# sparisi/pvr_habitat

Measured on AMD Instinct MI355X. Metric: frames/sec embedded (ResNet50, 256x256), higher is better.
Workload: dtype f16; 1 GPU; configs[1]: ResNet50 (MoCo-v2 layout) frozen, 256x256 uint8 frames resident in HBM, batch 256/GPU, random-init synthetic weights, f16 storage / MFMA inputs with fp32 accumulation (the product default, inside the 1e-3 parity bound; configs[1] names bf16); global_batch=256, frame=256, chunk=256, batches_in_flight=2, parallelism=frame shards, no collective (dp1)

## Files before the change

include/pvr_hip.h:

```cpp
#ifndef PVR_HIP_H
#define PVR_HIP_H

#include <stddef.h>
#include <stdint.h>

#ifdef __cplusplus
extern "C" {
#endif

typedef int pvr_status;
#define PVR_OK 0
#define PVR_ERR_INVALID 1
#define PVR_ERR_MISSING_WEIGHT 2
#define PVR_ERR_HIP 3
#define PVR_ERR_STATE 4

#define PVR_BF16 0
#define PVR_F16 1
#define PVR_F32 2

#define PVR_ARCH_RESNET50 0
#define PVR_ARCH_RESNET50_L4 1
#define PVR_ARCH_RESNET50_L3 2
#define PVR_ARCH_CLIP_VIT_B32 3
// ... 53 lines not shown
int32_t pvr_encoder_launch_kernel(const pvr_encoder *enc, int32_t n, int32_t index, char *buf, int32_t cap);
void pvr_encoder_destroy(pvr_encoder *enc);

pvr_status pvr_op_preprocess(const uint8_t *frames_dev, int32_t n, int32_t h, int32_t w, int32_t resize,
                             int32_t crop, void *out_dev, int32_t dtype, void *hip_stream);
pvr_status pvr_op_stem(const void *img_dev, const void *wgt_dev, const float *bias_dev, void *out_dev,
                       int32_t n, int32_t dtype, void *hip_stream);
pvr_status pvr_op_maxpool(const void *in_dev, void *out_dev, int32_t n, int32_t h, int32_t w, int32_t c,
                          int32_t dtype, void *hip_stream);
pvr_status pvr_op_conv2d(const void *in_dev, const void *wgt_dev, const float *bias_dev,
                         const void *residual_dev, void *out_dev, int32_t n, int32_t h, int32_t w,
                         int32_t cin, int32_t cout, int32_t kh, int32_t kw, int32_t stride, int32_t pad,
                         int32_t relu, int32_t out_f32, int32_t dtype, void *hip_stream);
pvr_status pvr_op_bneck_frame(const void *t1_dev, const void *w2_dev, const float *b2_dev, const void *w3_dev, const float *b3_dev,
                              const void *residual_dev, void *y_dev, void *t2_out_dev, const void *w1n_dev, const float *b1n_dev, void *t1n_dev,
                              const void *w1f_dev, const float *b1f_dev, int32_t n, int32_t phases, int32_t dtype, void *hip_stream);
pvr_status pvr_op_pack_frag_weights(const void *w_dev, void *out_dev, int32_t rows, int32_t k, void *hip_stream);
pvr_status pvr_debug_bneck_frame_stamps(const void *t1_dev, const void *w2_dev, const float *b2_dev, const void *w3_dev, const float *b3_dev,
                                        const void *residual_dev, void *y_dev, const void *w1n_dev, const float *b1n_dev, void *t1n_dev,
                                        const void *w1f_dev, const float *b1f_dev, int32_t n, int32_t dtype, uint64_t *stamps_dev, void *hip_stream);
int64_t pvr_debug_bneck_frame_launches(void);
pvr_status pvr_debug_set_frame64(int32_t mode);
int64_t pvr_debug_bneck_frame64_launches(void);
pvr_status pvr_debug_bneck_frame64_stamps(const void *w1f_dev, const float *b1f_dev, const void *w2_dev, const float *b2_dev, const void *w3_dev, const float *b3_dev,
                                          const void *x_dev, void *y_dev, int32_t n, int32_t dtype, uint64_t *stamps_dev, void *hip_stream);
pvr_status pvr_op_conv_wfrag(const void *in_dev, const void *wgt_packed_dev, const float *bias_dev, const void *residual_dev, void *out_dev, int32_t n,
                             int32_t h, int32_t w, int32_t cin, int32_t cout, int32_t kh, int32_t kw, int32_t stride, int32_t pad, int32_t relu,
                             int32_t out_f32, int32_t dtype, void *hip_stream);
pvr_status pvr_op_conv2d_dual(const void *in_dev, const void *in2_dev, const void *wgt_dev, const float *bias_dev, void *out_dev, int32_t n, int32_t h,
                              int32_t w, int32_t cin, int32_t cout, int32_t kh, int32_t kw, int32_t stride, int32_t pad, int32_t h2, int32_t w2,
                              int32_t cin2, int32_t stride2, int32_t relu, int32_t dtype, void *hip_stream);
pvr_status pvr_op_conv_wfrag_pool(const void *in_dev, const void *wgt_packed_dev, const float *bias_dev, const void *residual_dev, float *pool_out_dev,
                                  int64_t pool_stride, int32_t n, int32_t cin, int32_t cout, int32_t dtype, void *hip_stream);
int64_t pvr_debug_conv_wfrag_launches(void);
pvr_status pvr_op_split16_pack_weights(const float *w_dev, void *out_dev, int32_t rows, int32_t k, void *hip_stream);
pvr_status pvr_op_conv2d_split16(const float *in_dev, const void *wgt_split_dev, const float *bias_dev, const float *residual_dev, float *out_dev, int32_t n,
                                 int32_t h, int32_t w, int32_t cin, int32_t cout, int32_t k, int32_t stride, int32_t pad, int32_t relu, void *hip_stream);
pvr_status pvr_op_conv2d_f32(const float *in_dev, const float *wgt_dev, const float *bias_dev, const float *residual_dev, float *out_dev, int32_t n,
                             int32_t h, int32_t w, int32_t cin, int32_t cout, int32_t k, int32_t stride, int32_t pad, int32_t relu, void *hip_stream);
int64_t pvr_debug_conv_split16_launches(void);
int64_t pvr_debug_chain_wave128_launches(void);
pvr_status pvr_debug_set_conv_algo(int32_t algo);
pvr_status pvr_file_sizes(const char *const *paths, int32_t n, int64_t *sizes, int32_t threads);
pvr_status pvr_read_files(const char *const *paths, int32_t n, uint8_t *dst, const int64_t *offsets, int32_t threads);
pvr_status pvr_stage_copy(void *dst, const void *src, int64_t rows, int64_t row_bytes, int64_t src_row_stride, int64_t run_bytes,
                          int64_t run_stride, int32_t threads);
int64_t pvr_png_scratch_bytes(int32_t n, int32_t h, int32_t w);
pvr_status pvr_png_decode(const uint8_t *files_dev, const int64_t *offsets_dev, int32_t n, int32_t h, int32_t w, uint8_t *out_dev,
                          uint8_t *scratch_dev, int64_t scratch_bytes, int32_t *status_dev, void *hip_stream);

int64_t pvr_debug_conv_expand_launches(void);
int64_t pvr_debug_pp_persistent_launches(void);
pvr_status pvr_op_avgpool(const void *in_dev, float *out_dev, int64_t out_stride, int32_t n, int32_t hw,
                          int32_t c, int32_t in_f32, int32_t dtype, void *hip_stream);
pvr_status pvr_op_nonfinite_flag(const float *x_dev, int64_t rows, int64_t cols, int64_t stride, int32_t *flag_dev, void *hip_stream);

pvr_status pvr_op_attention(const void *qkv_dev, void *out_dev, int32_t T, int32_t W, int32_t heads, int32_t nb, int32_t dtype, void *hip_stream);
pvr_status pvr_op_layernorm(const float *x_dev, const float *patch_emb_dev, const float *cls_dev, const float *pos_dev, const float *gamma_dev,
                            const float *beta_dev, float *out_f32_dev, void *out_h_dev, int32_t rows, int32_t T, int32_t W, float eps, int32_t normalize,
                            int32_t dtype, void *hip_stream);
pvr_status pvr_op_cls_head(const float *x_dev, const float *gamma_dev, const float *beta_dev, const float *proj_or_null_dev, float *out_dev,
                           int64_t out_stride, int32_t nb, int32_t T, int32_t W, int32_t out_dim, float eps, void *hip_stream);

pvr_status pvr_debug_convert(const float *src, uint16_t *dst, int64_t n, int32_t dtype);


// ... 5 lines not shown
```

pvr_habitat_amd/_lib.py:

```python
import ctypes as C
import os

_HERE = os.path.dirname(os.path.abspath(__file__))
LIB_PATH = os.environ.get('PVR_LIB') or os.path.join(_HERE, 'lib', 'libpvr_hip.so')

PVR_BF16, PVR_F16, PVR_F32 = 0, 1, 2
ARCH_RESNET50, ARCH_RESNET50_L4, ARCH_RESNET50_L3 = 0, 1, 2


class EncoderDesc(C.Structure):
    _fields_ = [('arch', C.c_int32), ('dtype', C.c_int32), ('max_batch', C.c_int32), ('chunk', C.c_int32),
                ('resize', C.c_int32), ('crop', C.c_int32), ('mean', C.c_float * 3), ('std_', C.c_float * 3)]


_lib = None

_SIGS = {
    'pvr_version': (C.c_char_p, []),
    'pvr_has_experiments': (C.c_int32, []),
    'pvr_debug_stem_u8_geometry_ok': (C.c_int32, [C.c_void_p, C.c_int32, C.c_int32, C.c_int32, C.c_int32]),
    'pvr_encoder_set_host_backend': (C.c_int, [C.c_void_p, C.c_int32]),
    'pvr_stage_copy': (C.c_int, [C.c_void_p, C.c_void_p, C.c_int64, C.c_int64, C.c_int64, C.c_int64, C.c_int64, C.c_int32]),
    'pvr_last_error': (C.c_size_t, [C.c_char_p, C.c_size_t]),
    'pvr_encoder_create': (C.c_int, [C.POINTER(EncoderDesc), C.POINTER(C.c_void_p)]),
# ... 4 lines not shown
    'pvr_encoder_forward_lane': (C.c_int, [C.c_void_p, C.c_int32, C.c_void_p, C.c_int32, C.c_int32, C.c_int32, C.c_void_p, C.c_int64, C.c_void_p]),
    'pvr_debug_set_conv_algo': (C.c_int, [C.c_int32]),
    'pvr_file_sizes': (C.c_int, [C.c_void_p, C.c_int32, C.c_void_p, C.c_int32]),
    'pvr_read_files': (C.c_int, [C.c_void_p, C.c_int32, C.c_void_p, C.c_void_p, C.c_int32]),
    'pvr_png_scratch_bytes': (C.c_int64, [C.c_int32, C.c_int32, C.c_int32]),
    'pvr_png_decode': (C.c_int, [C.c_void_p, C.c_void_p, C.c_int32, C.c_int32, C.c_int32, C.c_void_p, C.c_void_p, C.c_int64, C.c_void_p, C.c_void_p]),
    'pvr_debug_conv_expand_launches': (C.c_int64, []),
    'pvr_debug_pp_persistent_launches': (C.c_int64, []),
    'pvr_encoder_set_crop_position': (C.c_int, [C.c_void_p, C.c_int32]),
    'pvr_encoder_set_low_latency': (C.c_int, [C.c_void_p, C.c_int32]),
    'pvr_encoder_tap': (C.c_int, [C.c_void_p, C.c_char_p, C.c_void_p, C.c_int64, C.POINTER(C.c_int64), C.c_void_p]),
    'pvr_encoder_debug_stop_after': (C.c_int, [C.c_void_p, C.c_char_p]),
    'pvr_encoder_debug_set_fusion': (C.c_int, [C.c_void_p, C.c_int32]),
    'pvr_encoder_launch_name': (C.c_int32, [C.c_void_p, C.c_int32, C.c_char_p, C.c_int32]),
    'pvr_encoder_destroy': (None, [C.c_void_p]),
    'pvr_encoder_profile': (C.c_int, [C.c_void_p, C.c_void_p, C.c_int32, C.c_int32, C.c_int32, C.c_void_p, C.c_int64, C.c_void_p,
                                      C.c_void_p, C.c_void_p, C.c_int32, C.POINTER(C.c_int32)]),
    'pvr_encoder_profile_span': (C.c_int, [C.c_void_p, C.c_void_p, C.c_int32, C.c_int32, C.c_int32, C.c_void_p, C.c_int64, C.c_void_p, C.c_int32, C.c_int32,
                                           C.POINTER(C.c_float)]),
    'pvr_op_preprocess': (C.c_int, [C.c_void_p, C.c_int32, C.c_int32, C.c_int32, C.c_int32, C.c_int32, C.c_void_p, C.c_int32, C.c_void_p]),
    'pvr_op_stem': (C.c_int, [C.c_void_p, C.c_void_p, C.c_void_p, C.c_void_p, C.c_int32, C.c_int32, C.c_void_p]),
    'pvr_op_maxpool': (C.c_int, [C.c_void_p, C.c_void_p, C.c_int32, C.c_int32, C.c_int32, C.c_int32, C.c_int32, C.c_void_p]),
    'pvr_op_conv2d': (C.c_int, [C.c_void_p, C.c_void_p, C.c_void_p, C.c_void_p, C.c_void_p] + [C.c_int32] * 12 + [C.c_void_p]),
    'pvr_op_avgpool': (C.c_int, [C.c_void_p, C.c_void_p, C.c_int64, C.c_int32, C.c_int32, C.c_int32, C.c_int32, C.c_int32, C.c_void_p]),
    'pvr_debug_convert': (C.c_int, [C.c_void_p, C.c_void_p, C.c_int64, C.c_int32]),
    'pvr_op_bneck_frame': (C.c_int, [C.c_void_p] * 13 + [C.c_int32] * 3 + [C.c_void_p]),
    'pvr_debug_bneck_frame_launches': (C.c_int64, []),
    'pvr_debug_set_frame64': (C.c_int, [C.c_int32]),
    'pvr_debug_bneck_frame64_launches': (C.c_int64, []),
    'pvr_debug_bneck_frame64_stamps': (C.c_int, [C.c_void_p] * 8 + [C.c_int32] * 2 + [C.c_void_p] * 2),
    'pvr_op_conv_wfrag': (C.c_int, [C.c_void_p] * 5 + [C.c_int32] * 12 + [C.c_void_p]),
    'pvr_debug_conv_wfrag_launches': (C.c_int64, []),
    'pvr_op_conv_wfrag_pool': (C.c_int, [C.c_void_p] * 5 + [C.c_int64] + [C.c_int32] * 4 + [C.c_void_p]),
    'pvr_op_conv2d_dual': (C.c_int, [C.c_void_p] * 5 + [C.c_int32] * 15 + [C.c_void_p]),
    'pvr_op_pack_frag_weights': (C.c_int, [C.c_void_p, C.c_void_p, C.c_int32, C.c_int32, C.c_void_p]),
    'pvr_debug_bneck_frame_stamps': (C.c_int, [C.c_void_p] * 12 + [C.c_int32] * 2 + [C.c_void_p] * 2),
    'pvr_encoder_check_range': (C.c_int, [C.c_void_p, C.c_void_p, C.c_int32, C.c_int32, C.c_int32, C.c_void_p, C.c_int64, C.c_void_p, C.POINTER(C.c_int32)]),
    'pvr_encoder_debug_set_switch': (C.c_int, [C.c_void_p, C.c_char_p, C.c_int32]),
    'pvr_encoder_launch_kernel': (C.c_int32, [C.c_void_p, C.c_int32, C.c_int32, C.c_char_p, C.c_int32]),
    'pvr_op_split16_pack_weights': (C.c_int, [C.c_void_p, C.c_void_p, C.c_int32, C.c_int32, C.c_void_p]),
    'pvr_op_conv2d_split16': (C.c_int, [C.c_void_p] * 5 + [C.c_int32] * 9 + [C.c_void_p]),
    'pvr_op_conv2d_f32': (C.c_int, [C.c_void_p] * 5 + [C.c_int32] * 9 + [C.c_void_p]),
    'pvr_debug_conv_split16_launches': (C.c_int64, []),
    'pvr_debug_chain_wave128_launches': (C.c_int64, []),
    'pvr_op_attention': (C.c_int, [C.c_void_p, C.c_void_p, C.c_int32, C.c_int32, C.c_int32, C.c_int32, C.c_int32, C.c_void_p]),
    'pvr_op_layernorm': (C.c_int, [C.c_void_p] * 8 + [C.c_int32] * 3 + [C.c_float, C.c_int32, C.c_int32, C.c_void_p]),
    'pvr_op_cls_head': (C.c_int, [C.c_void_p] * 5 + [C.c_int64] + [C.c_int32] * 4 + [C.c_float, C.c_void_p]),
    'pvr_op_nonfinite_flag': (C.c_int, [C.c_void_p, C.c_int64, C.c_int64, C.c_int64, C.c_void_p, C.c_void_p]),
}


def lib():
    global _lib
    if _lib is None:
        if not os.path.isfile(LIB_PATH):
            raise RuntimeError('libpvr_hip.so not found at %s: build it with `make -C pvr_habitat_amd/csrc` '
                               '(there is no CPU fallback for the HIP path)' % LIB_PATH)
        l = C.CDLL(LIB_PATH)
        for name, (res, args) in _SIGS.items():
            if not hasattr(l, name):
                continue
            f = getattr(l, name)
            f.restype, f.argtypes = res, args
        _lib = l
    return _lib

# ... 22 lines not shown
```

pvr_habitat_amd/csrc/api.hip:

```cpp
#include <stdarg.h>
#include "encoder_internal.h"
#include "sample_rng.h"
#include <dlfcn.h>

namespace pvr {

static thread_local std::string g_err;

void set_error(const char *fmt, ...) {
    char buf[1024];
    va_list ap;
    va_start(ap, fmt);
    vsnprintf(buf, sizeof buf, fmt, ap);
    va_end(ap);
    g_err = buf;
}
const std::string &last_error() { return g_err; }

namespace {
typedef int (*roctx_push_fn)(const char *);
typedef int (*roctx_pop_fn)();
struct Roctx {
    roctx_push_fn push = nullptr;
    roctx_pop_fn pop = nullptr;
// ... 65 lines not shown
                              w1n, b1n, t1n, w1f, b1f);
}
pvr_status pvr_debug_set_frame64(int32_t mode) {
    PVR_REQUIRE(mode >= -1 && mode <= 1, "pvr_debug_set_frame64: -1 (environment: PVR_FRAME64, default off), 0 or 1");
    if (mode < 0) { PlanSwitches env; read_switches(env); mode = env.frame64; }
    op_switches().frame64 = mode;
    return PVR_OK;
}
int64_t pvr_debug_bneck_frame64_launches(void) { return (int64_t)bneck_frame64_launches(); }
pvr_status pvr_debug_bneck_frame64_stamps(const void *w1f, const float *b1f, const void *w2, const float *b2, const void *w3, const float *b3, const void *x, void *y,
                                          int32_t n, int32_t dtype, uint64_t *stamps_dev, void *stream) {
    PVR_REQUIRE(stamps_dev && n > 8, "pvr_debug_bneck_frame64_stamps: needs a stamp buffer and more than 8 frames");
    return launch_bneck_frame64(w1f, b1f, w2, b2, w3, b3, x, y, n, dtype, (hipStream_t)stream, (unsigned long long *)stamps_dev);
}
pvr_status pvr_op_conv_wfrag(const void *in, const void *wgt_packed, const float *bias, const void *residual, void *out, int32_t n, int32_t h, int32_t w,
                             int32_t cin, int32_t cout, int32_t kh, int32_t kw, int32_t stride, int32_t pad, int32_t relu, int32_t out_f32, int32_t dtype,
                             void *stream) {
    PVR_REQUIRE(n > 0 && h > 0 && w > 0, "pvr_op_conv_wfrag: empty input");
    return launch_conv_wfrag(op_switches(), in, wgt_packed, bias, residual, out, n, h, w, cin, cout, kh, kw, stride, pad, relu, out_f32, dtype, (hipStream_t)stream);
}
pvr_status pvr_op_conv2d_dual(const void *in, const void *in2, const void *wgt, const float *bias, void *out, int32_t n, int32_t h, int32_t w, int32_t cin,
                              int32_t cout, int32_t kh, int32_t kw, int32_t stride, int32_t pad, int32_t h2, int32_t w2, int32_t cin2, int32_t stride2,
                              int32_t relu, int32_t dtype, void *stream) {
    PVR_REQUIRE(in && in2 && wgt && bias && out && n > 0, "pvr_op_conv2d_dual: null argument");
    PVR_REQUIRE(dtype == PVR_BF16 || dtype == PVR_F16, "pvr_op_conv2d_dual: 16-bit storage types only");
    return launch_conv_pp256(op_switches(), in, wgt, bias, nullptr, out, n, h, w, cin, cout, kh, kw, stride, pad, relu, 0, 0, dtype, 224, (hipStream_t)stream, in2, h2, w2,
                             cin2, stride2);
}
pvr_status pvr_op_conv_wfrag_pool(const void *in, const void *wgt_packed, const float *bias, const void *residual, float *pool_out, int64_t pool_stride,
                                  int32_t n, int32_t cin, int32_t cout, int32_t dtype, void *stream) {
    PVR_REQUIRE(n > 0 && pool_out, "pvr_op_conv_wfrag_pool: empty input");
    return launch_conv_wfrag(op_switches(), in, wgt_packed, bias, residual, nullptr, n, 7, 7, cin, cout, 1, 1, 1, 0, 1, 1, dtype, (hipStream_t)stream, pool_out, pool_stride);
}
int64_t pvr_debug_conv_wfrag_launches(void) { return (int64_t)conv_wfrag_launches(); }
pvr_status pvr_op_split16_pack_weights(const float *w, void *out, int32_t rows, int32_t k, void *stream) {
    return launch_split16_pack(w, out, rows, k, (hipStream_t)stream);
}
pvr_status pvr_op_conv2d_split16(const float *in, const void *wgt_split, const float *bias, const float *residual, float *out, int32_t n, int32_t h,
                                 int32_t w, int32_t cin, int32_t cout, int32_t k, int32_t stride, int32_t pad, int32_t relu, void *stream) {
    PVR_REQUIRE(n > 0 && h > 0 && w > 0, "pvr_op_conv2d_split16: empty input");
    return launch_conv_split16(in, wgt_split, bias, residual, out, n, h, w, cin, cout, k, stride, pad, relu, (hipStream_t)stream);
}
pvr_status pvr_op_conv2d_f32(const float *in, const float *wgt, const float *bias, const float *residual, float *out, int32_t n, int32_t h, int32_t w,
                             int32_t cin, int32_t cout, int32_t k, int32_t stride, int32_t pad, int32_t relu, void *stream) {
    PVR_REQUIRE(in && wgt && bias && out && n > 0, "pvr_op_conv2d_f32: null argument");
    return launch_conv_f32(in, wgt, bias, residual, out, n, h, w, cin, cout, k, stride, pad, relu, (hipStream_t)stream);
}
int64_t pvr_debug_conv_split16_launches(void) { return (int64_t)conv_split16_launches(); }
int64_t pvr_debug_chain_wave128_launches(void) { return (int64_t)chain_wave128_launches(); }
int64_t pvr_debug_pp_persistent_launches(void) { return (int64_t)pp_persistent_launches(); }

size_t pvr_last_error(char *buf, size_t cap) {
    const std::string &e = last_error();
    if (buf && cap) {
        size_t n = e.size() < cap - 1 ? e.size() : cap - 1;
        memcpy(buf, e.data(), n);
        buf[n] = 0;
    }
    return e.size();
}

pvr_status pvr_op_preprocess(const uint8_t *frames, int32_t n, int32_t h, int32_t w, int32_t resize, int32_t crop,
                             void *out, int32_t dtype, void *stream) {
    PVR_REQUIRE(frames && out, "pvr_op_preprocess: null pointer");
    hipStream_t st = (hipStream_t)stream;
    PVR_HIP_TRY(hipMemsetAsync(out, 0, (size_t)n * (crop + 6) * (crop + 8) * 4 * 2, st));
// ... 95 lines not shown
```

pvr_habitat_amd/csrc/conv_wfrag.hip:

```cpp
#include "encoder_internal.h"

namespace pvr {

struct WFP {
    const u16 *in, *w, *res;
    const float *bias;
    void *out;
    int M, H, W, Cin, Cout, Ho, Wo, KH, KW, stride, pad, act;
    int MT, NCT;
    int nch, cpt;
    int KC;
    int ct_major;
    unsigned in_bytes, w_bytes, out_bytes, res_bytes;
    float *pool_out;
    long long pool_stride;
    int frames;
};

#define WF_LDS_PTR(off_) ((__attribute__((address_space(3))) void *)(smem + (off_)))

template <bool F16, int RES, bool OUT32, int KO = 0, bool POOL = false>
__global__ __launch_bounds__(512, 1) void conv_wfrag_kernel(WFP p) {
    typedef typename HT<F16>::V8 V8;
    constexpr int BMV = POOL ? 98 : 112;
    constexpr int BM = 112, NT = 7, XB = 16384;
    constexpr int OOB = 0x7ffffff0;
    extern __shared__ __attribute__((aligned(16))) char smem[];

    const int tid = threadIdx.x, lane = tid & 63;
    const int wave = __builtin_amdgcn_readfirstlane(tid >> 6);
    const int fr = lane & 15, fq = lane >> 4, sw = (fr >> 1) & 7;
    const int t = xcd_remap(blockIdx.x, gridDim.x);
    int mt, ct;
    if (p.ct_major) { ct = t / p.MT; mt = t - ct * p.MT; }
    else { mt = t / p.NCT; ct = t - mt * p.NCT; }
    const int m0 = mt * BMV, co0 = ct * 256;

    const auto rs_in = __builtin_amdgcn_make_buffer_rsrc(const_cast<u16 *>(p.in), 0, p.in_bytes, 0x00020000);
    const auto rs_w = __builtin_amdgcn_make_buffer_rsrc(const_cast<u16 *>(p.w), 0, p.w_bytes, 0x00020000);

    int a_off[2], a_m[2];
#pragma unroll
    for (int i = 0; i < 2; ++i) {
        const int g = wave + 8 * i, r = g * 8 + (lane >> 3);
        const int lch = (lane & 7) ^ ((r >> 1) & 7);
        const int m = m0 + r;
        const bool ok = g < BM / 8 && r < BMV && m < p.M;
        const int mm = ok ? m : 0;
        const int wo = mm % p.Wo, tq = mm / p.Wo, ho = tq % p.Ho, n = tq / p.Ho;
// ... 163 lines not shown
    if constexpr (POOL) {
#pragma unroll
        for (int f = 0; f < 2; ++f) {
            float tot[8];
#pragma unroll
            for (int e = 0; e < 8; ++e) {
                float t = ps[f][e];
                if (f == 1) t = __builtin_bit_cast(float, __builtin_amdgcn_update_dpp(0, __builtin_bit_cast(int, t), 0x12f, 0xf, 0xf, false));
                t += __builtin_bit_cast(float, __builtin_amdgcn_update_dpp(0, __builtin_bit_cast(int, t), 0x111, 0xf, 0xf, true));
                t += __builtin_bit_cast(float, __builtin_amdgcn_update_dpp(0, __builtin_bit_cast(int, t), 0x112, 0xf, 0xf, true));
                t += __builtin_bit_cast(float, __builtin_amdgcn_update_dpp(0, __builtin_bit_cast(int, t), 0x114, 0xf, 0xf, true));
                t += __builtin_bit_cast(float, __builtin_amdgcn_update_dpp(0, __builtin_bit_cast(int, t), 0x118, 0xf, 0xf, true));
                tot[e] = t / 49.f;
            }
            const int frame = 2 * mt + f;
            if (fr == 15 && frame < p.frames) {
                float *o = p.pool_out + (long long)frame * p.pool_stride + c;
                *reinterpret_cast<f32x4 *>(o) = f32x4{tot[0], tot[1], tot[2], tot[3]};
                *reinterpret_cast<f32x4 *>(o + 4) = f32x4{tot[4], tot[5], tot[6], tot[7]};
            }
        }
    }
#undef WF_ITER
#undef WF_STEP
#undef WF_XREAD
#undef WF_LOAD_W1
#undef WF_LOAD_W_
#undef WF_LOAD_W
#undef WF_STAGE
#undef WF_STAGE1
#undef WF_STAGE_NEXT
}

static long long g_conv_wfrag_launches = 0;
long long conv_wfrag_launches() { return g_conv_wfrag_launches; }

bool conv_wfrag_supported(int64_t M, int64_t in_bytes, int cin, int cout, int kh, int kw, int pad, int act, int out_f32) {
    const int64_t K = (int64_t)kh * kw * cin;
    return cin % 64 == 0 && cout % 256 == 0 && kh <= 3 && kh == kw && (pad == kh / 2 || pad == 0) && (act == 0 || act == 1) && !(out_f32 & 2) && M >= 1 &&
           M * cout * ((out_f32 & 1) ? 4 : 2) < 0x7ffffff0ll && in_bytes < 0x7ffffff0ll && (int64_t)cout * K * 2 < 0x7ffffff0ll;
}

bool conv_wfrag_preferred(const PlanSwitches &sw, int64_t M, int cin, int cout, int kh, int kw) {
    const int on = sw.conv_wfrag;
    const int64_t K = (int64_t)kh * kw * cin, nct = cout / 256, t256 = ((M + 255) / 256) * nct, t112 = ((M + 111) / 112) * nct;
    if (on == 2) return K >= 512;
    return on && K >= 1024 && t256 < 160 && t112 >= 192;
}

pvr_status launch_conv_wfrag(const PlanSwitches &sw, const void *in, const void *wp, const float *bias, const void *res, void *out, int n, int h, int w, int cin, int cout,
                             int kh, int kw, int stride, int pad, int act, int out_f32, int dtype, hipStream_t stream, float *pool_out, int64_t pool_stride) {
    PVR_REQUIRE(in && wp && bias && (out || pool_out), "conv_wfrag: null argument");
    PVR_REQUIRE(dtype == PVR_BF16 || dtype == PVR_F16, "conv_wfrag: 16-bit storage types only");
    const int ho = (h + 2 * pad - kh) / stride + 1, wo = (w + 2 * pad - kw) / stride + 1;
    const int64_t M = (int64_t)n * ho * wo;
    PVR_REQUIRE(conv_wfrag_supported(M, (int64_t)n * h * w * cin * 2, cin, cout, kh, kw, pad, act, out_f32), "conv_wfrag: unsupported shape");
    WFP p;
    p.in = (const u16 *)in; p.w = (const u16 *)wp; p.res = (const u16 *)res; p.bias = bias; p.out = out;
    p.M = (int)M; p.H = h; p.W = w; p.Cin = cin; p.Cout = cout; p.Ho = ho; p.Wo = wo; p.KH = kh; p.KW = kw; p.stride = stride; p.pad = pad; p.act = act;
    p.MT = pool_out ? (n + 1) / 2 : (int)((M + 111) / 112); p.NCT = cout / 256;
    p.pool_out = pool_out; p.pool_stride = pool_stride; p.frames = n;
    PVR_REQUIRE(!pool_out || (ho == 7 && wo == 7 && res && act == 1 && pool_stride >= cout && ((size_t)pool_out & 15) == 0 && pool_stride % 4 == 0),
                "conv_wfrag: the pooled form is the 7 x 7 conv3 + identity + ReLU of the trunk's last block");
    p.cpt = cin / 64; p.nch = kh * kw * p.cpt; p.KC = kh * kw * cin / 8;
    const int64_t wbytes = (int64_t)cout * kh * kw * cin * 2;
    p.ct_major = wbytes > (5 << 19) ? 1 : 0;
    p.in_bytes = (unsigned)((int64_t)n * h * w * cin * 2); p.w_bytes = (unsigned)wbytes;
    p.out_bytes = (unsigned)(M * cout * ((out_f32 & 1) ? 4 : 2)); p.res_bytes = res ? (unsigned)(M * cout * 2) : 0;
    constexpr int lds = 4 * 16384;
    const dim3 grid((unsigned)(p.MT * p.NCT)), block(512);
    ++g_conv_wfrag_launches;
    const bool f16 = dtype == PVR_F16, o32 = out_f32 & 1;
#define WF_GO(F_, R_, O_) hipLaunchKernelGGL((conv_wfrag_kernel<F_, R_, O_>), grid, block, lds, stream, p)
#ifdef PVR_EXPERIMENTS
    if (sw.wfrag_ko && dtype == PVR_F16 && !res && !(out_f32 & 1)) {
#define WF_KO(k_) case k_: hipLaunchKernelGGL((conv_wfrag_kernel<true, 0, false, k_>), grid, block, lds, stream, p); break;
        switch (sw.wfrag_ko) { WF_KO(1) WF_KO(2) WF_KO(3) WF_KO(4) WF_KO(7) WF_KO(8) WF_KO(9) WF_KO(10) WF_KO(11) WF_KO(15) default: break; }
#undef WF_KO
        PVR_LAUNCH_CHECK();
        return PVR_OK;
    }
#endif
    if (pool_out) {
        if (f16) hipLaunchKernelGGL((conv_wfrag_kernel<true, 1, false, 0, true>), grid, block, lds, stream, p);
        else hipLaunchKernelGGL((conv_wfrag_kernel<false, 1, false, 0, true>), grid, block, lds, stream, p);
        PVR_LAUNCH_CHECK();
        return PVR_OK;
    }
    if (f16) {
        if (res) { if (o32) WF_GO(true, 1, true); else WF_GO(true, 1, false); }
        else { if (o32) WF_GO(true, 0, true); else WF_GO(true, 0, false); }
    } else {
        if (res) { if (o32) WF_GO(false, 1, true); else WF_GO(false, 1, false); }
        else { if (o32) WF_GO(false, 0, true); else WF_GO(false, 0, false); }
    }
#undef WF_GO
    PVR_LAUNCH_CHECK();
    return PVR_OK;
}

}
```

pvr_habitat_amd/csrc/encoder.hip:

```cpp
#include "encoder_internal.h"

namespace pvr {

pvr_status launch_split16_pack(const float *w, void *out, int rows, int K, hipStream_t stream);
pvr_status launch_conv_split16(const float *in, const void *wsp, const float *bias, const float *res, float *out, int n, int h, int w, int cin,
                               int cout, int k, int stride, int pad, int relu, hipStream_t stream, float *out2 = nullptr, int n1 = 0, void *out16 = nullptr,
                               int terms = 3);

void read_switches(PlanSwitches &sw) {
    auto get = [](const char *name, int def) { const char *v = getenv(name); return v ? atoi(v) : def; };
    sw.pool_fuse = get("PVR_POOL_FUSE", 1);
    sw.stem_u8 = get("PVR_STEM_U8", 1);
    sw.stem_lds = get("PVR_STEM_LDS", 1);
    sw.stem_regpool = get("PVR_STEM_REGPOOL", 1);
    sw.frame_front1 = get("PVR_FRAME_FRONT1", 1);
    sw.frame_next1 = get("PVR_FRAME_NEXT1", 0);
    sw.frame_bneck = get("PVR_FRAME_BNECK", 1);
    sw.frame64 = get("PVR_FRAME64", 0);
    sw.bneck_stagger = get("PVR_FRAME_STAGGER", 0);
    sw.dual_ds = get("PVR_DUAL_DS", 1);
    sw.chain_ds = get("PVR_CHAIN_DS", 1);
    sw.chain_blocked = get("PVR_CHAIN_BLOCKED", 1);
    sw.chain_halo = get("PVR_CHAIN_HALO", 1);
    sw.chain_ds_occ = get("PVR_CHAIN_DS_OCC", 3);
    sw.chain_pfk = get("PVR_CHAIN_PFK", 12);
    sw.chain_cfg = get("PVR_CHAIN_CFG", 12);
    sw.chain_wave = get("PVR_CHAIN_WAVE", 1);
    sw.chain_wave_halo = get("PVR_CHAIN_WAVE_HALO", 1);
    sw.chain_wave_128 = get("PVR_CHAIN_WAVE_128", 1);
    sw.strided_y = get("PVR_STRIDED_Y", 1);
    sw.chain_wave_l2 = get("PVR_CHAIN_WAVE_L2", 0);
    sw.splitk = get("PVR_SPLITK", 1);
    sw.smallk_div = get("PVR_SMALLK_DIV", 4);
    if (sw.smallk_div < 1) sw.smallk_div = 1;
    sw.frame_min_n = get("PVR_FRAME_MIN_N", 128);
    sw.frame_run = get("PVR_FRAME_RUN", 0);
    sw.frame_stagger = get("PVR_FRAME_RUN_STAGGER", 0);
    sw.split16 = get("PVR_SPLIT16", 1);
    sw.stem_conv1 = get("PVR_STEM_CONV1", 1);
    sw.resid32 = get("PVR_RESID32", 1);
    sw.tail_f32 = get("PVR_TAIL_F32", 1);
    sw.fuse = get("PVR_FUSE", 1);
    sw.conv_algo = get("PVR_CONV_ALGO", -1);
    sw.conv_halo = get("PVR_CONV_HALO", 1);
// ... 811 lines not shown
    PVR_REQUIRE(pos >= 0 && pos <= 4, "crop position %d outside 0..4", pos);
    PVR_REQUIRE(pos == 0 || (!enc->vit && !enc->rnd && enc->desc.arch != PVR_ARCH_CLIP_RN50), "corner crops are built for the ResNet50 family only");
    enc->crop_pos = pos;
    return PVR_OK;
}

pvr_status pvr_encoder_set_low_latency(pvr_encoder *enc, int32_t on) {
    PVR_REQUIRE(enc, "null encoder");
    enc->low_latency = on != 0;
    if (enc->vit || enc->rnd || enc->host) return PVR_OK;
    resolve_kinds(enc);
    if (!enc->finalized) return PVR_OK;
    return ensure_smallk(enc);
}

pvr_status pvr_encoder_debug_set_fusion(pvr_encoder *enc, int32_t on) {
    PVR_REQUIRE(enc, "null encoder");
    enc->fuse = on != 0;
    if (!enc->vit && !enc->rnd && !enc->host) resolve_kinds(enc);
    return PVR_OK;
}

pvr_status pvr_encoder_debug_set_switch(pvr_encoder *enc, const char *name, int32_t value) {
    PVR_REQUIRE(enc && name, "pvr_encoder_debug_set_switch: null argument");
    const std::string nm = name;
    if (nm == "pool_fuse") enc->sw.pool_fuse = value;
    else if (nm == "stem_u8") enc->sw.stem_u8 = value;
    else if (nm == "frame_min_n") enc->sw.frame_min_n = value;
    else if (nm == "frame_run") enc->sw.frame_run = value;
    else if (nm == "frame_stagger") enc->sw.frame_stagger = value;
    else if (nm == "conv_algo") enc->sw.conv_algo = value;
    else if (nm == "frame64") enc->sw.frame64 = value;
    else if (nm == "stem_regpool") enc->sw.stem_regpool = value;
    else {
        set_error("pvr_encoder_debug_set_switch: '%s' is not a live switch (pool_fuse, stem_u8, frame_min_n, frame_run, frame_stagger, conv_algo, frame64, "
                  "stem_regpool); plan switches are read from the environment at create", name);
        return PVR_ERR_INVALID;
    }
    if (!enc->vit && !enc->rnd && !enc->host) resolve_kinds(enc);
    return PVR_OK;
}

pvr_status pvr_encoder_check_range(pvr_encoder *enc, const uint8_t *frames, int32_t n, int32_t h, int32_t w, float *out, int64_t out_stride, void *hip_stream,
                                   int32_t *first_bad) {
    PVR_REQUIRE(enc && frames && out && first_bad, "pvr_encoder_check_range: null argument");
    PVR_NO_HOST(enc, "pvr_encoder_check_range");
    PVR_REQUIRE(enc->finalized && !enc->vit && !enc->rnd && enc->desc.arch != PVR_ARCH_CLIP_RN50 && enc->desc.dtype != PVR_F32,
                "pvr_encoder_check_range: built for the 16-bit plans of the torchvision ResNet family");
    PVR_REQUIRE(n > 0 && n <= enc->desc.chunk, "pvr_encoder_check_range: n=%d must fit one chunk (%d)", n, enc->desc.chunk);
    hipStream_t st = (hipStream_t)hip_stream;
    const size_t nl = enc->sched_plain.size();
    pvr_status s = use_lane(enc, 0);
    if (!s) s = lane_wait(enc, 0, hip_stream);
    if (s) return s;
    int *flags = nullptr;
    PVR_HIP_TRY(hipMalloc((void **)&flags, (nl + 1) * sizeof(int)));
    if (hipMemsetAsync(flags, 0, (nl + 1) * sizeof(int), st) != hipSuccess) { (void)hipFree(flags); set_error("check_range: memset failed"); return PVR_ERR_HIP; }
    const bool fuse0 = enc->fuse;
    enc->fuse = false; resolve_kinds(enc);
    enc->range_flags = flags;
    s = forward_impl(enc, frames, n, h, w, out, out_stride, hip_stream, nullptr);
    enc->range_flags = nullptr;
    enc->fuse = fuse0; resolve_kinds(enc);
    std::vector<int> hf(nl + 1, 0);
    if (!s && hipMemcpyAsync(hf.data(), flags, (nl + 1) * sizeof(int), hipMemcpyDeviceToHost, st) != hipSuccess) { set_error("check_range: copy failed"); s = PVR_ERR_HIP; }
    if (!s && hipStreamSynchronize(st) != hipSuccess) { set_error("check_range: sync failed"); s = PVR_ERR_HIP; }
    (void)hipFree(flags);
    if (s) return s;
    *first_bad = hf[nl] ? 1 : -1;
// ... 86 lines not shown
```

pvr_habitat_amd/csrc/encoder_internal.h:

```cpp
#pragma once
#include <map>
#include <string>
#include <vector>
#include <cmath>
#include "common.h"
#include "chain_params.h"

namespace pvr {

struct PlanSwitches {
    int pool_fuse = 1;
    int stem_u8 = 1;
    int stem_lds = 1;
    int stem_regpool = 1;
    int frame_front1 = 1;
    int frame_next1 = 0;
    int frame_bneck = 1;
    int frame64 = 0;
    int bneck_stagger = 0;
    int dual_ds = 1;
    int chain_ds = 1;
    int chain_blocked = 1;
    int chain_halo = 1;
    int chain_ds_occ = 3;
    int chain_pfk = 12;
    int chain_cfg = 12;
    int chain_wave = 1;
    int chain_wave_halo = 1;
    int chain_wave_128 = 1;
    int chain_wave_l2 = 0;
    int strided_y = 1;
    int splitk = 1;
    int smallk_div = 4;
    int frame_run = 0;
    int frame_stagger = 0;
    int frame_min_n = 128;
    int stem_conv1 = 1;
    int split16 = 1;
    int resid32 = 1;
    int tail_f32 = 1;
    int fuse = 1;
    int conv_algo = -1;
    int conv_halo = 1;
    int conv_expand = 1;
// ... 25 lines not shown
pvr_status launch_conv_splitk(const void *, const void *, const float *, const void *, void *, const void *, float *, int, int, int, int, int, int,
                              int, int, int, int, int, int, int, hipStream_t);
pvr_status launch_conv(const PlanSwitches &sw, const void *, const void *, const float *, const void *, void *, const void *, int, int, int, int,
                       int, int, int, int, int, int, int, int, hipStream_t);

bool conv_expand_supported(const PlanSwitches &sw, int64_t M, int h, int w, int cin, int cout, int kh, int kw, int stride, int pad, int relu, int out_f32, bool has_res);
pvr_status launch_conv_expand(const void *in, const void *wgt, const float *bias, const void *res, void *out, int n, int h, int w, int cin,
                              int cout, int stride, int relu, int dtype, hipStream_t stream, int out_blk = 0);

bool pp256_supported(int64_t M, int cin, int cout, int kh, int kw, int64_t in_bytes, int64_t w_bytes, int64_t out_bytes, int64_t res_bytes);
pvr_status launch_conv_pp256(const PlanSwitches &sw, const void *in, const void *wgt, const float *bias, const void *res, void *out, int n, int h, int w, int cin,
                             int cout, int kh, int kw, int stride, int pad, int act, int out_f32, int res_f32, int dtype, int bm, hipStream_t stream,
                             const void *in2 = nullptr, int h2 = 0, int w2 = 0, int cin2 = 0, int stride2 = 1);

bool bneck_frame_supported(const PlanSwitches &sw, int n, int h, int w, int cm, int cout, int stride);
pvr_status launch_pack_frag_weights(const void *w, void *out, int rows, int K, hipStream_t stream);
pvr_status launch_bneck_frame(const PlanSwitches &sw, const void *t1, const void *w2p, const float *b2, const void *w3p, const float *b3, const void *res, void *y,
                              void *t2_out, int n, int phases, int dtype, hipStream_t stream, unsigned long long *stamps = nullptr,
                              const void *w1np = nullptr, const float *b1n = nullptr, void *t1n = nullptr, const void *w1fp = nullptr, const float *b1f = nullptr);
struct BFBlk {
    const unsigned short *w1f, *w2, *w3, *res;
    const float *b1f, *b2, *b3;
    unsigned short *y;
};
pvr_status launch_bneck_frame_run(const BFBlk *blocks, int nblk, int n, int dtype, hipStream_t stream, int stagger);
pvr_status launch_bneck_frame64(const void *w1p, const float *b1, const void *w2p, const float *b2, const void *w3p, const float *b3, const void *x, void *y, int n,
                                int dtype, hipStream_t stream, unsigned long long *stamps);
long long bneck_frame64_launches();

bool conv_wfrag_supported(int64_t M, int64_t in_bytes, int cin, int cout, int kh, int kw, int pad, int act, int out_f32);
bool conv_wfrag_preferred(const PlanSwitches &sw, int64_t M, int cin, int cout, int kh, int kw);
pvr_status launch_conv_wfrag(const PlanSwitches &sw, const void *in, const void *wp, const float *bias, const void *res, void *out, int n, int h, int w, int cin, int cout,
                             int kh, int kw, int stride, int pad, int act, int out_f32, int dtype, hipStream_t stream, float *pool_out = nullptr,
                             int64_t pool_stride = 0);

struct HostTensor {
    std::vector<int64_t> shape;
    std::vector<float> data;
};

constexpr int PVR_MAX_LANES = 4;
enum BufId { B_NONE = -1, B_X0 = 0, B_X1, B_T1, B_T2, B_DS, B_F32, B_Y0, B_Y1, B_COUNT, B_STEM = B_COUNT };

struct ConvOp {
    std::string conv, bn;
    int in_buf, out_buf, res_buf;
    int h, w, cin, cin_real, cout, cout_real, k, stride, pad, relu, out_f32;
    int kind = 0;
    bool f32op = false;
    bool from32 = false;
    bool split16 = false;
    bool wfrag = false;
    u16 *d_w = nullptr;
    u16 *d_wp = nullptr;
    u16 *d_wfb = nullptr;
    u16 *d_wpb = nullptr;
    std::vector<u16> h_w;
    float *d_wf = nullptr;
    u16 *d_wpk = nullptr;
    u16 *d_wsp_pair = nullptr;
    float *d_b_pair = nullptr;
    u16 *d_wsp = nullptr;
    float *d_b = nullptr;
    std::vector<float> h_b;
    float *d_bsum = nullptr;
    u16 *d_wcat = nullptr;
    std::string tap;
// ... 138 lines not shown
```

Measured before the change: 101,400 frames/s.

## Add input-resident pooled conv kernel looping over several output-channel tiles per workgroup

Adds a new kernel for the final 1x1 conv3 + identity + ReLU + avgpool layer. Each workgroup keeps its two-frame input slab resident in LDS and loops over T output-channel tiles, instead of one tile per workgroup. This is meant to avoid re-staging the same input for every channel tile and to size the grid to the CU count. The cost is fewer workgroups and less latency hiding, plus complex hand-scheduled wait counts that could stall or be fragile.

```diff
diff --git a/include/pvr_hip.h b/include/pvr_hip.h
--- a/include/pvr_hip.h
+++ b/include/pvr_hip.h
@@ -109,6 +109,9 @@
                               int32_t cin2, int32_t stride2, int32_t relu, int32_t dtype, void *hip_stream);
 pvr_status pvr_op_conv_wfrag_pool(const void *in_dev, const void *wgt_packed_dev, const float *bias_dev, const void *residual_dev, float *pool_out_dev,
                                   int64_t pool_stride, int32_t n, int32_t cin, int32_t cout, int32_t dtype, void *hip_stream);
+pvr_status pvr_op_conv_wfrag_pool_tiles(const void *in_dev, const void *wgt_packed_dev, const float *bias_dev, const void *residual_dev, float *pool_out_dev,
+                                        int64_t pool_stride, int32_t n, int32_t cin, int32_t cout, int32_t dtype, void *hip_stream, int32_t tiles_per_wg);
+int32_t pvr_debug_conv_wfrag_pool_tiles(int32_t n, int32_t cout, int32_t cus);
 int64_t pvr_debug_conv_wfrag_launches(void);
 pvr_status pvr_op_split16_pack_weights(const float *w_dev, void *out_dev, int32_t rows, int32_t k, void *hip_stream);
 pvr_status pvr_op_conv2d_split16(const float *in_dev, const void *wgt_split_dev, const float *bias_dev, const float *residual_dev, float *out_dev, int32_t n,
diff --git a/pvr_habitat_amd/_lib.py b/pvr_habitat_amd/_lib.py
--- a/pvr_habitat_amd/_lib.py
+++ b/pvr_habitat_amd/_lib.py
@@ -60,6 +60,8 @@
     'pvr_op_conv_wfrag': (C.c_int, [C.c_void_p] * 5 + [C.c_int32] * 12 + [C.c_void_p]),
     'pvr_debug_conv_wfrag_launches': (C.c_int64, []),
     'pvr_op_conv_wfrag_pool': (C.c_int, [C.c_void_p] * 5 + [C.c_int64] + [C.c_int32] * 4 + [C.c_void_p]),
+    'pvr_op_conv_wfrag_pool_tiles': (C.c_int, [C.c_void_p] * 5 + [C.c_int64] + [C.c_int32] * 4 + [C.c_void_p] + [C.c_int32]),
+    'pvr_debug_conv_wfrag_pool_tiles': (C.c_int32, [C.c_int32] * 3),
     'pvr_op_conv2d_dual': (C.c_int, [C.c_void_p] * 5 + [C.c_int32] * 15 + [C.c_void_p]),
     'pvr_op_pack_frag_weights': (C.c_int, [C.c_void_p, C.c_void_p, C.c_int32, C.c_int32, C.c_void_p]),
     'pvr_debug_bneck_frame_stamps': (C.c_int, [C.c_void_p] * 12 + [C.c_int32] * 2 + [C.c_void_p] * 2),
diff --git a/pvr_habitat_amd/csrc/api.hip b/pvr_habitat_amd/csrc/api.hip
--- a/pvr_habitat_amd/csrc/api.hip
+++ b/pvr_habitat_amd/csrc/api.hip
@@ -121,6 +121,13 @@
     PVR_REQUIRE(n > 0 && pool_out, "pvr_op_conv_wfrag_pool: empty input");
     return launch_conv_wfrag(op_switches(), in, wgt_packed, bias, residual, nullptr, n, 7, 7, cin, cout, 1, 1, 1, 0, 1, 1, dtype, (hipStream_t)stream, pool_out, pool_stride);
 }
+pvr_status pvr_op_conv_wfrag_pool_tiles(const void *in, const void *wgt_packed, const float *bias, const void *residual, float *pool_out, int64_t pool_stride,
+                                        int32_t n, int32_t cin, int32_t cout, int32_t dtype, void *stream, int32_t tiles_per_wg) {
+    PVR_REQUIRE(n > 0 && pool_out, "pvr_op_conv_wfrag_pool_tiles: empty input");
+    return launch_conv_wfrag(op_switches(), in, wgt_packed, bias, residual, nullptr, n, 7, 7, cin, cout, 1, 1, 1, 0, 1, 1, dtype, (hipStream_t)stream, pool_out, pool_stride,
+                             tiles_per_wg);
+}
+int32_t pvr_debug_conv_wfrag_pool_tiles(int32_t n, int32_t cout, int32_t cus) { return n > 0 && cout >= 256 && cus > 0 ? conv_wfrag_pool_tiles(n, cout, cus) : 1; }
 int64_t pvr_debug_conv_wfrag_launches(void) { return (int64_t)conv_wfrag_launches(); }
 pvr_status pvr_op_split16_pack_weights(const float *w, void *out, int32_t rows, int32_t k, void *stream) {
     return launch_split16_pack(w, out, rows, k, (hipStream_t)stream);
diff --git a/pvr_habitat_amd/csrc/conv_wfrag.hip b/pvr_habitat_amd/csrc/conv_wfrag.hip
--- a/pvr_habitat_amd/csrc/conv_wfrag.hip
+++ b/pvr_habitat_amd/csrc/conv_wfrag.hip
@@ -15,6 +15,7 @@
     float *pool_out;
     long long pool_stride;
     int frames;
+    int T;
 };
 
 #define WF_LDS_PTR(off_) ((__attribute__((address_space(3))) void *)(smem + (off_)))
@@ -244,6 +245,214 @@
 #undef WF_STAGE_NEXT
 }
 
+constexpr int rs_idn(int nch, int s) { return nch == 8 ? (s < 3 ? 3 : 0) : (s == 0 ? 9 : 0); }
+constexpr int rs_later(int nch, int s) {
+    if (nch != 8) return 8;
+    int n = 8;
+    for (int d = 1; d <= 3; ++d) n += rs_idn(8, (s + 8 - d) & 7);
+    return n;
+}
+constexpr int rs_first(int nch, int s) { return nch != 8 ? 8 : s == 0 ? 20 : s == 1 ? 21 : s == 2 ? 22 : rs_later(8, s); }
+
+template <bool F16, int NCH>
+__global__ __launch_bounds__(512, 1) void conv_wfrag_pool_resident_kernel(WFP p) {
+    typedef typename HT<F16>::V8 V8;
+    constexpr int BMV = 98, NT = 7, XB = 16384, OOB = 0x7ffffff0;
+    constexpr int WROW = NCH * 2048;
+    static_assert(NCH == 1 || NCH == 2 || NCH == 4 || NCH == 8, "chunk positions and weight sets must line up: NCH divides 4 or is 8");
+    extern __shared__ __attribute__((aligned(16))) char smem[];
+
+    const int tid = threadIdx.x, lane = tid & 63;
+    const int wave = __builtin_amdgcn_readfirstlane(tid >> 6);
+    const int fr = lane & 15, fq = lane >> 4, sw = (fr >> 1) & 7;
+    const int t = xcd_remap(blockIdx.x, gridDim.x);
+    const int T = p.T, cg = t / p.MT, mt = t - cg * p.MT;
+    const int m0 = mt * BMV, co_first = cg * T * 256;
+    const bool two = 2 * mt + 1 < p.frames;
+
+    const auto rs_in = __builtin_amdgcn_make_buffer_rsrc(const_cast<u16 *>(p.in), 0, p.in_bytes, 0x00020000);
+    const auto rs_w = __builtin_amdgcn_make_buffer_rsrc(const_cast<u16 *>(p.w), 0, p.w_bytes, 0x00020000);
+    const auto rs_r = __builtin_amdgcn_make_buffer_rsrc(const_cast<u16 *>(p.res), 0, p.res_bytes, 0x00020000);
+    const auto rs_b = __builtin_amdgcn_make_buffer_rsrc(const_cast<float *>(p.bias), 0, p.Cout * 4, 0x00020000);
+
+    int a_v[2];
+#pragma unroll
+    for (int i = 0; i < 2; ++i) {
+        const int g = wave + 8 * i, r = g * 8 + (lane >> 3);
+        const int lch = (lane & 7) ^ ((r >> 1) & 7);
+        const int m = m0 + r;
+        a_v[i] = (g < 14 && r < BMV && m < p.M) ? (m * p.Cin + lch * 8) * 2 : OOB;
+    }
+#define RS_STAGE(c_)                                                                                            \
+    {                                                                                                          \
+        __builtin_amdgcn_raw_ptr_buffer_load_lds(rs_in, WF_LDS_PTR((c_) * XB + wave * 1024), 16, a_v[0], (c_) * 128, 0, 0);         \
+        __builtin_amdgcn_raw_ptr_buffer_load_lds(rs_in, WF_LDS_PTR((c_) * XB + (wave + 8) * 1024), 16, a_v[1], (c_) * 128, 0, 0);   \
+        asm volatile("" ::: "memory");                                                                          \
+    }
+    const int wlane = lane * 16;
+    const int wbase = ((co_first >> 4) + 2 * wave) * WROW;
+    int tile = 0;
+    V8 w0[2][2], w1[2][2], w2[2][2], w3[2][2];
+#define RS_WOFF(i_, ks_, tt_, cc_) (wbase + (tile + (tt_) < T ? tile + (tt_) : T - 1) * (16 * WROW) + (i_) * WROW + (2 * (cc_) + (ks_)) * 1024)
+#define RS_LOAD_W1(dst_, i_, ks_, tt_, cc_)                                                                     \
+    {                                                                                                          \
+        dst_[i_][ks_] = __builtin_bit_cast(V8, __builtin_amdgcn_raw_buffer_load_b128(rs_w, wlane, RS_WOFF(i_, ks_, tt_, cc_), 0));   \
+        asm volatile("" ::: "memory");                                                                          \
+    }
+#define RS_LOAD_W(dst_, f_) { RS_LOAD_W1(dst_, 0, 0, (f_) / NCH, (f_) % NCH) RS_LOAD_W1(dst_, 0, 1, (f_) / NCH, (f_) % NCH)   \
+                              RS_LOAD_W1(dst_, 1, 0, (f_) / NCH, (f_) % NCH) RS_LOAD_W1(dst_, 1, 1, (f_) / NCH, (f_) % NCH) }
+
+    const int cl = co_first + 32 * wave + 8 * fq;
+    const int ro = ((m0 + fr) * p.Cout + cl) * 2, bo = cl * 4;
+    const int ro3 = (fr == 0 || two) ? ro : OOB, ro45 = two ? ro : OOB, ro6 = (two && fr < 2) ? ro : OOB;
+    u32x4 rr[NT], bb[2];
+#define RS_IDREQ(k_)                                                                                            \
+    {                                                                                                          \
+        if constexpr ((k_) < 7)                                                                                 \
+            rr[(k_) < 7 ? (k_) : 0] = __builtin_bit_cast(u32x4, __builtin_amdgcn_raw_buffer_load_b128(rs_r, (k_) < 3 ? ro : (k_) == 3 ? ro3 : (k_) < 6 ? ro45 : ro6, \
+                                                                                                   (k_) * 32 * p.Cout + tile * 512, 0));     \
+        else                                                                                                    \
+            bb[(k_) < 7 ? 0 : (k_) - 7] = __builtin_bit_cast(u32x4, __builtin_amdgcn_raw_buffer_load_b128(rs_b, bo, tile * 1024 + ((k_) - 7) * 16, 0));   \
+        asm volatile("" ::: "memory");                                                                          \
+    }
+#define RS_ID(s_, q_)                                                                                           \
+    {                                                                                                          \
+        if constexpr (NCH == 8) { if constexpr ((s_) < 3 && (q_) >= 4) RS_IDREQ(3 * (s_) + (q_) - 4) }          \
+        else if constexpr ((s_) == 0) { RS_IDREQ(q_) if constexpr ((q_) >= 5) RS_IDREQ((q_) + 2) }              \
+    }
+
+    f32x4 acc[2][NT];
+#pragma unroll
+    for (int i = 0; i < 2; ++i)
+#pragma unroll
+        for (int j = 0; j < NT; ++j) acc[i][j] = f32x4{0.f, 0.f, 0.f, 0.f};
+
+    const int xc = fr * 128 + ((fq ^ sw) << 4), xc64 = xc ^ 64, xh = xc + 4 * XB, xh64 = xc64 + 4 * XB;
+    V8 xs[NT][2];
+    constexpr int RD = 3;
+#define RS_XREAD(j_, B_)                                                                                        \
+    {                                                                                                          \
+        asm volatile("ds_read_b128 %0, %1 offset:%2" : "=v"(xs[j_][0]) : "v"((B_) < 4 ? xc : xh), "n"(((B_) & 3) * XB + (j_) * 2048));     \
+        asm volatile("ds_read_b128 %0, %1 offset:%2" : "=v"(xs[j_][1]) : "v"((B_) < 4 ? xc64 : xh64), "n"(((B_) & 3) * XB + (j_) * 2048)); \
+    }
+#define RS_STEP(q_, B_, BN_, W_)                                                                                \
+    {                                                                                                          \
+        if ((q_) + RD < NT) RS_XREAD((q_) + RD, B_) else RS_XREAD((q_) + RD - NT, BN_);                         \
+        asm volatile("s_waitcnt lgkmcnt(6)" : "+v"(xs[q_][0]), "+v"(xs[q_][1]));                                \
+        __builtin_amdgcn_sched_barrier(0);                                                                      \
+        acc[0][q_] = mfma16<F16>(W_[0][0], xs[q_][0], acc[0][q_]);                                              \
+        acc[1][q_] = mfma16<F16>(W_[1][0], xs[q_][0], acc[1][q_]);                                              \
+        acc[0][q_] = mfma16<F16>(W_[0][1], xs[q_][1], acc[0][q_]);                                              \
+        acc[1][q_] = mfma16<F16>(W_[1][1], xs[q_][1], acc[1][q_]);                                              \
+    }
+#define RS_ITER(u_, W_, WF_)                                                                                    \
+    {                                                                                                          \
+        constexpr int s_ = (u_) % NCH, sn_ = (s_ + 1) % NCH, tt_ = (s_ + 3) / NCH, cc_ = (s_ + 3) % NCH;        \
+        if ((u_) < NCH && tile == 0) {                                                                          \
+            asm volatile("s_waitcnt vmcnt(%0)" :: "n"(rs_first(NCH, s_)) : "memory");                           \
+            if constexpr (NCH == 8 ? s_ <= 3 : s_ + 1 < NCH) __builtin_amdgcn_s_barrier();                      \
+        } else {                                                                                                \
+            asm volatile("s_waitcnt vmcnt(%0)" :: "n"(rs_later(NCH, s_)) : "memory");                           \
+        }                                                                                                       \
+        __builtin_amdgcn_sched_barrier(0);                                                                      \
+        RS_LOAD_W1(WF_, 0, 0, tt_, cc_) RS_ID(s_, 0) RS_STEP(0, s_, sn_, W_)                                    \
+        RS_LOAD_W1(WF_, 0, 1, tt_, cc_) RS_ID(s_, 1) RS_STEP(1, s_, sn_, W_)                                    \
+        RS_LOAD_W1(WF_, 1, 0, tt_, cc_) RS_ID(s_, 2) RS_STEP(2, s_, sn_, W_)                                    \
+        RS_LOAD_W1(WF_, 1, 1, tt_, cc_) RS_ID(s_, 3) RS_STEP(3, s_, sn_, W_)                                    \
+        RS_ID(s_, 4) RS_STEP(4, s_, sn_, W_)                                                                    \
+        RS_ID(s_, 5) RS_STEP(5, s_, sn_, W_)                                                                    \
+        RS_ID(s_, 6) RS_STEP(6, s_, sn_, W_)                                                                    \
+    }
+
+    auto epilogue = [&]() {
+        asm volatile("s_waitcnt lgkmcnt(0)" : "+v"(xs[0][0]), "+v"(xs[0][1]), "+v"(xs[1][0]), "+v"(xs[1][1]), "+v"(xs[2][0]), "+v"(xs[2][1]));
+        __builtin_amdgcn_sched_barrier(0);
+        const int c = cl + tile * 256;
+        const f32x4 bl = __builtin_bit_cast(f32x4, bb[0]), bh = __builtin_bit_cast(f32x4, bb[1]);
+        float ps[2][8];
+#pragma unroll
+        for (int f = 0; f < 2; ++f)
+#pragma unroll
+            for (int e = 0; e < 8; ++e) ps[f][e] = 0.f;
+#pragma unroll
+        for (int j = 0; j < NT; ++j) {
+            const f32x4 lo = acc[0][j], hi = acc[1][j];
+            float v[8] = {lo[0] + bl[0], lo[1] + bl[1], lo[2] + bl[2], lo[3] + bl[3], hi[0] + bh[0], hi[1] + bh[1], hi[2] + bh[2], hi[3] + bh[3]};
+#pragma unroll
+            for (int e = 0; e < 4; ++e) {
+                v[2 * e] += from_h<F16>((u16)(rr[j][e] & 0xffffu));
+                v[2 * e + 1] += from_h<F16>((u16)(rr[j][e] >> 16));
+            }
+#pragma unroll
+            for (int e = 0; e < 8; ++e) v[e] = fmaxf(v[e], 0.f);
+            const int pp = 16 * j + fr;
+#pragma unroll
+            for (int e = 0; e < 8; ++e) {
+                ps[0][e] += pp < 49 ? v[e] : 0.f;
+                ps[1][e] += (pp >= 49 && pp < 98) ? v[e] : 0.f;
+            }
+            acc[0][j] = f32x4{0.f, 0.f, 0.f, 0.f};
+            acc[1][j] = f32x4{0.f, 0.f, 0.f, 0.f};
+        }
+#pragma unroll
+        for (int f = 0; f < 2; ++f) {
+            float tot[8];
+#pragma unroll
+            for (int e = 0; e < 8; ++e) {
+                float s = ps[f][e];
+                if (f == 1) s = __builtin_bit_cast(float, __builtin_amdgcn_update_dpp(0, __builtin_bit_cast(int, s), 0x12f, 0xf, 0xf, false));
+                s += __builtin_bit_cast(float, __builtin_amdgcn_update_dpp(0, __builtin_bit_cast(int, s), 0x111, 0xf, 0xf, true));
+                s += __builtin_bit_cast(float, __builtin_amdgcn_update_dpp(0, __builtin_bit_cast(int, s), 0x112, 0xf, 0xf, true));
+                s += __builtin_bit_cast(float, __builtin_amdgcn_update_dpp(0, __builtin_bit_cast(int, s), 0x114, 0xf, 0xf, true));
+                s += __builtin_bit_cast(float, __builtin_amdgcn_update_dpp(0, __builtin_bit_cast(int, s), 0x118, 0xf, 0xf, true));
+                tot[e] = s / 49.f;
+            }
+            const int frame = 2 * mt + f;
+            if (fr == 15 && frame < p.frames) {
+                float *o = p.pool_out + (long long)frame * p.pool_stride + c;
+                *reinterpret_cast<f32x4 *>(o) = f32x4{tot[0], tot[1], tot[2], tot[3]};
+                *reinterpret_cast<f32x4 *>(o + 4) = f32x4{tot[4], tot[5], tot[6], tot[7]};
+            }
+        }
+    };
+#define RS_END(u_) { if constexpr (((u_) + 1) % NCH == 0) { epilogue(); if (++tile >= T) break; } }
+
+    RS_STAGE(0) RS_LOAD_W(w0, 0)
+    if constexpr (NCH > 1) RS_STAGE(1)
+    RS_LOAD_W(w1, 1)
+    if constexpr (NCH > 2) RS_STAGE(2)
+    RS_LOAD_W(w2, 2)
+    if constexpr (NCH > 3) RS_STAGE(3)
+    if constexpr (NCH > 4) { RS_STAGE(4) RS_STAGE(5) RS_STAGE(6) RS_STAGE(7) }
+    asm volatile("s_waitcnt vmcnt(%0)" :: "n"(12 + 2 * (NCH - 1)) : "memory");
+    __builtin_amdgcn_s_barrier();
+    __builtin_amdgcn_sched_barrier(0);
+    RS_XREAD(0, 0) RS_XREAD(1, 0) RS_XREAD(2, 0)
+#pragma unroll 1
+    for (;;) {
+        RS_ITER(0, w0, w3) RS_END(0)
+        RS_ITER(1, w1, w0) RS_END(1)
+        RS_ITER(2, w2, w1) RS_END(2)
+        RS_ITER(3, w3, w2) RS_END(3)
+        if constexpr (NCH == 8) {
+            RS_ITER(4, w0, w3)
+            RS_ITER(5, w1, w0)
+            RS_ITER(6, w2, w1)
+            RS_ITER(7, w3, w2) RS_END(7)
+        }
+    }
+#undef RS_END
+#undef RS_ITER
+#undef RS_STEP
+#undef RS_XREAD
+#undef RS_ID
+#undef RS_IDREQ
+#undef RS_LOAD_W
+#undef RS_LOAD_W1
+#undef RS_WOFF
+#undef RS_STAGE
+}
+
 static long long g_conv_wfrag_launches = 0;
 long long conv_wfrag_launches() { return g_conv_wfrag_launches; }
 
@@ -260,8 +469,39 @@
     return on && K >= 1024 && t256 < 160 && t112 >= 192;
 }
 
+int conv_wfrag_pool_tiles(int n, int cout, int cus) {
+    const int64_t nct = cout / 256, mt = ((int64_t)n + 1) / 2;
+    for (int T = 4; T > 1; T >>= 1)
+        if (nct % T == 0 && mt * (nct / T) >= cus) return T;
+    return 1;
+}
+
+static int wf_num_cus() {
+    static int v = 0;
+    if (!v) {
+        int dev = 0, n = 0;
+        if (hipGetDevice(&dev) == hipSuccess && hipDeviceGetAttribute(&n, hipDeviceAttributeMultiprocessorCount, dev) == hipSuccess && n > 0) v = n;
+        else v = 256;
+    }
+    return v;
+}
+
+template <bool F16, int NCH>
+static pvr_status launch_pool_resident(const WFP &p, hipStream_t stream) {
+    constexpr int lds = NCH * 16384;
+    static DeviceOnce attr_done;
+    if (attr_done.needed()) {
+        PVR_HIP_TRY(hipFuncSetAttribute((const void *)conv_wfrag_pool_resident_kernel<F16, NCH>, hipFuncAttributeMaxDynamicSharedMemorySize, lds));
+        attr_done.mark();
+    }
+    hipLaunchKernelGGL((conv_wfrag_pool_resident_kernel<F16, NCH>), dim3((unsigned)(p.MT * (p.NCT / p.T))), dim3(512), lds, stream, p);
+    PVR_LAUNCH_CHECK();
+    return PVR_OK;
+}
+
 pvr_status launch_conv_wfrag(const PlanSwitches &sw, const void *in, const void *wp, const float *bias, const void *res, void *out, int n, int h, int w, int cin, int cout,
-                             int kh, int kw, int stride, int pad, int act, int out_f32, int dtype, hipStream_t stream, float *pool_out, int64_t pool_stride) {
+                             int kh, int kw, int stride, int pad, int act, int out_f32, int dtype, hipStream_t stream, float *pool_out, int64_t pool_stride,
+                             int pool_tiles) {
     PVR_REQUIRE(in && wp && bias && (out || pool_out), "conv_wfrag: null argument");
     PVR_REQUIRE(dtype == PVR_BF16 || dtype == PVR_F16, "conv_wfrag: 16-bit storage types only");
     const int ho = (h + 2 * pad - kh) / stride + 1, wo = (w + 2 * pad - kw) / stride + 1;
@@ -271,7 +511,7 @@
     p.in = (const u16 *)in; p.w = (const u16 *)wp; p.res = (const u16 *)res; p.bias = bias; p.out = out;
     p.M = (int)M; p.H = h; p.W = w; p.Cin = cin; p.Cout = cout; p.Ho = ho; p.Wo = wo; p.KH = kh; p.KW = kw; p.stride = stride; p.pad = pad; p.act = act;
     p.MT = pool_out ? (n + 1) / 2 : (int)((M + 111) / 112); p.NCT = cout / 256;
-    p.pool_out = pool_out; p.pool_stride = pool_stride; p.frames = n;
+    p.pool_out = pool_out; p.pool_stride = pool_stride; p.frames = n; p.T = 1;
     PVR_REQUIRE(!pool_out || (ho == 7 && wo == 7 && res && act == 1 && pool_stride >= cout && ((size_t)pool_out & 15) == 0 && pool_stride % 4 == 0),
                 "conv_wfrag: the pooled form is the 7 x 7 conv3 + identity + ReLU of the trunk's last block");
     p.cpt = cin / 64; p.nch = kh * kw * p.cpt; p.KC = kh * kw * cin / 8;
@@ -294,6 +534,17 @@
     }
 #endif
     if (pool_out) {
+        PVR_REQUIRE(pool_tiles == 0 || ((pool_tiles == 1 || pool_tiles == 2 || pool_tiles == 4) && p.NCT % pool_tiles == 0),
+                    "conv_wfrag: tiles per workgroup must be 0 (the launcher's rule), 1, 2 or 4 and divide cout / 256");
+        p.T = pool_tiles ? pool_tiles : sw.wfrag_pool_resident ? conv_wfrag_pool_tiles(n, cout, wf_num_cus()) : 1;
+        if (p.T > 1 && kh == 1 && (p.nch == 1 || p.nch == 2 || p.nch == 4 || p.nch == 8)) {
+            switch (p.nch) {
+            case 1: return f16 ? launch_pool_resident<true, 1>(p, stream) : launch_pool_resident<false, 1>(p, stream);
+            case 2: return f16 ? launch_pool_resident<true, 2>(p, stream) : launch_pool_resident<false, 2>(p, stream);
+            case 4: return f16 ? launch_pool_resident<true, 4>(p, stream) : launch_pool_resident<false, 4>(p, stream);
+            default: return f16 ? launch_pool_resident<true, 8>(p, stream) : launch_pool_resident<false, 8>(p, stream);
+            }
+        }
         if (f16) hipLaunchKernelGGL((conv_wfrag_kernel<true, 1, false, 0, true>), grid, block, lds, stream, p);
         else hipLaunchKernelGGL((conv_wfrag_kernel<false, 1, false, 0, true>), grid, block, lds, stream, p);
         PVR_LAUNCH_CHECK();
diff --git a/pvr_habitat_amd/csrc/encoder.hip b/pvr_habitat_amd/csrc/encoder.hip
--- a/pvr_habitat_amd/csrc/encoder.hip
+++ b/pvr_habitat_amd/csrc/encoder.hip
@@ -10,6 +10,7 @@
 void read_switches(PlanSwitches &sw) {
     auto get = [](const char *name, int def) { const char *v = getenv(name); return v ? atoi(v) : def; };
     sw.pool_fuse = get("PVR_POOL_FUSE", 1);
+    sw.wfrag_pool_resident = get("PVR_WFRAG_POOL_RESIDENT", 1);
     sw.stem_u8 = get("PVR_STEM_U8", 1);
     sw.stem_lds = get("PVR_STEM_LDS", 1);
     sw.stem_regpool = get("PVR_STEM_REGPOOL", 1);
@@ -887,9 +888,10 @@
     else if (nm == "conv_algo") enc->sw.conv_algo = value;
     else if (nm == "frame64") enc->sw.frame64 = value;
     else if (nm == "stem_regpool") enc->sw.stem_regpool = value;
+    else if (nm == "wfrag_pool_resident") enc->sw.wfrag_pool_resident = value;
     else {
         set_error("pvr_encoder_debug_set_switch: '%s' is not a live switch (pool_fuse, stem_u8, frame_min_n, frame_run, frame_stagger, conv_algo, frame64, "
-                  "stem_regpool); plan switches are read from the environment at create", name);
+                  "stem_regpool, wfrag_pool_resident); plan switches are read from the environment at create", name);
         return PVR_ERR_INVALID;
     }
     if (!enc->vit && !enc->rnd && !enc->host) resolve_kinds(enc);
diff --git a/pvr_habitat_amd/csrc/encoder_internal.h b/pvr_habitat_amd/csrc/encoder_internal.h
--- a/pvr_habitat_amd/csrc/encoder_internal.h
+++ b/pvr_habitat_amd/csrc/encoder_internal.h
@@ -10,6 +10,7 @@
 
 struct PlanSwitches {
     int pool_fuse = 1;
+    int wfrag_pool_resident = 1;
     int stem_u8 = 1;
     int stem_lds = 1;
     int stem_regpool = 1;
@@ -101,7 +102,8 @@
 bool conv_wfrag_preferred(const PlanSwitches &sw, int64_t M, int cin, int cout, int kh, int kw);
 pvr_status launch_conv_wfrag(const PlanSwitches &sw, const void *in, const void *wp, const float *bias, const void *res, void *out, int n, int h, int w, int cin, int cout,
                              int kh, int kw, int stride, int pad, int act, int out_f32, int dtype, hipStream_t stream, float *pool_out = nullptr,
-                             int64_t pool_stride = 0);
+                             int64_t pool_stride = 0, int pool_tiles = 0);
+int conv_wfrag_pool_tiles(int n, int cout, int cus);
 
 struct HostTensor {
     std::vector<int64_t> shape;
```

After: 101,500 frames/s (median of 6 runs). Within noise of the previous version (+0.1%).
